# XinShuo-ph/gaussian_splatting_with_eye_tracking

Hardware: AMD Instinct MI355X
Metric: rendered views/sec (fwd+bwd) at 1080p, 1M Gaussians; achieved HBM GB/s % (higher is better)
Workload: dtype fp32; 1 GPU

## Files before the change

gaussian_splatting_with_eye_tracking_amd/csrc/gs_api.cpp:

```cpp
#include <hip/hip_runtime.h>

#include <atomic>
#include <cstdio>
#include <cstdlib>
#include <chrono>
#include <cstring>
#include <functional>
#include <algorithm>
#include <deque>
#include <mutex>
#include <stdexcept>
#include <string>
#include <unordered_set>
#include <utility>
#include <vector>

#include "../../include/gsplat_amd.h"
#include "gs_kernels.h"
#include "gs_layout.h"

using namespace gsamd;

namespace {

// ... 310 lines not shown
    in.store_cov3d = t_store_cov3d != 0;
    in.fwd_zero = t_fwd_zero != 0 && grad;
    in.step0_unfilled = amr && t_amr_step0_unfilled != 0;
    if (amr) t_amr_step0_unfilled = 0;
    return in;
}

PreprocessArgs make_pp(const ForwardIn& in, int tile) {
    PreprocessArgs a;
    a.P = in.P;
    a.D = in.D;
    a.M = in.M;
    a.means3D = in.means3D;
    a.scales = in.scales;
    a.scale_modifier = in.scale_modifier;
    a.rotations = in.rotations;
    a.opacities = in.opacities;
    a.shs = in.shs;
    a.cov3D_precomp = in.cov3D_precomp;
    a.colors_precomp = in.colors_precomp;
    a.viewmatrix = in.viewmatrix;
    a.projmatrix = in.projmatrix;
    a.cam_pos = in.cam_pos;
    a.W = in.width;
    a.H = in.height;
    a.tan_fovx = in.tan_fovx;
    a.tan_fovy = in.tan_fovy;
    a.focal_y = (float)in.height / (2.0f * in.tan_fovy);
    a.focal_x = (float)in.width / (2.0f * in.tan_fovx);
    a.block = tile;
    a.prefiltered = in.prefiltered;
    a.store_cov3d = in.store_cov3d;
    a.store_drgb = in.store_drgb;
    a.zero_words = nullptr;
    a.zero_n = 0;
    a.err_token = 0;
    a.antialiasing = in.antialiasing;
    return a;
}

struct Binned {
    GeomView g;
    ImageView img;
    BinningView b;
    AmrBinningView ab;
    int K;
    int T;
    int* radii;
};

int tile_count(int W, int H, int tile) { return ((W + tile - 1) / tile) * ((H + tile - 1) / tile); }

ImageView image_view(char* image, int W, int H, int tile) {
    ImageView v;
    carve_image(image, (size_t)W * H, tile_count(W, H, tile), &v, tile);
    return v;
}

Binned carve_buffers(char* geom, char* binning, char* image, int P, int K, int W, int H, int tile,
                     bool amr = false) {
    Binned r{};
    r.K = K;
    r.T = tile_count(W, H, tile);
    carve_geom(geom, P, &r.g);
    r.img = image_view(image, W, H, tile);
    carve_binning(binning, K, &r.b, amr ? &r.ab : nullptr);
    r.radii = r.g.radii;
    return r;
}

int rendered_count(int hint, char* geom, int P, const char* binning, hipStream_t s, const char* missing) {
    int K = hint;
    if (K < 0) {
        GeomView g;
        carve_geom(geom, P, &g);
        uint32_t hdr[4];
        read_header(g.hdr, hdr, s);
        K = (int)hdr[kHdrNumRendered];
    }
    if (K > 0 && !binning) throw GsError(missing);
    return K;
}

Binned preprocess_and_bin(const ForwardIn& in, const gs_buffer& geometry, const gs_buffer& binning,
                          const gs_buffer& image, int* radii, int tile, bool debug, hipStream_t s,
                          const std::function<void(Binned&)>& before_k = nullptr, int fused_sort_max = 0) {
    Binned r;
    const int W = in.width, H = in.height;
    const int gx = (W + tile - 1) / tile, gy = (H + tile - 1) / tile;
    r.T = gx * gy;
    const size_t N = (size_t)W * H;
    const bool tail = in.store_cov3d || (in.colors_precomp == nullptr && in.store_drgb);
    char* gbase = call_resize(geometry, carve_geom(nullptr, in.P, nullptr, tail, tile == 32), "geometry");
    carve_geom(gbase, in.P, &r.g);
    set_accum_clean(r.g.grad_accum, false);
    char* ibase = call_resize(image, carve_image(nullptr, N, r.T, nullptr, tile), "image");
    carve_image(ibase, N, r.T, &r.img, tile);
    r.radii = radii ? radii : r.g.radii;
    const bool lds_bin = r.T <= kLdsTiles;
    if (r.T == 0) GS_HIP(hipMemsetAsync(r.g.hdr, 0, kHdrWords * sizeof(uint32_t), s));
    if (r.T > 0 && !lds_bin) GS_HIP(hipMemsetAsync(r.img.tile_count, 0, sizeof(uint32_t) * kBinSlots * r.T, s));
    PreprocessArgs pa = make_pp(in, tile);
    pa.err_token = next_error_token();
    set_drgb_written(r.g.drgb, pa.store_drgb && in.colors_precomp == nullptr);
    if (r.T > 0 && lds_bin) {
        pa.zero_words = r.img.tile_count;
        pa.zero_n = kBinSlots * r.T;
    }
    { StageTimer _t(kPre, s); launch_preprocess(pa, r.g, r.radii, lds_bin ? nullptr : r.img.tile_count, s); }
    stage_check(debug, s, "preprocess");
    if (lds_bin) { StageTimer _t(kCount, s); launch_count_tiles(in.P, r.g, r.radii, W, H, tile, r.img, s); }
    stage_check(debug, s, "count_tiles");
    const std::pair<uint32_t*, uint32_t*> mirror =
        (r.T > 0 && hdr_mirror_on()) ? mirror_words() : std::pair<uint32_t*, uint32_t*>{nullptr, nullptr};
    const bool amr = tile == 32;
    bool dup_done = false;
    const SpecKey skey = spec_key(W, H, in.P);
    const size_t cap = (!amr && !before_k && r.T > 0 && !debug) ? spec_capacity(skey) : 0;
    const uint32_t mtoken = mirror.second ? next_mirror_token() : 0u;
    const bool pub_dup = cap > 0 && mirror.second != nullptr;
    if (r.T > 0) { StageTimer _t(kScan, s); launch_tile_scan(r.T, r.img, r.g.hdr, s, pub_dup ? nullptr : mirror.second, bin_slots_for(in.P, gx, gy, tile), gx, dup_banded(gx, gy, tile), pub_dup ? 0u : mtoken); }
    stage_check(debug, s, "tile_scan");
    uint32_t hdr[4];
    if (before_k) {
        begin_header_read(r.g.hdr, s, mirror.first);
        before_k(r);
        finish_header_read(hdr, mirror.first, s, r.g.hdr);
    } else if (cap > 0) {
        begin_header_read(r.g.hdr, s, mirror.first);
        char* sbase = call_resize(binning, carve_binning(nullptr, cap, nullptr), "binning");
        carve_binning(sbase, cap, &r.b);
        { StageTimer _t(kDup, s); launch_duplicate(in.P, r.g, r.radii, W, H, tile, r.img, r.b, s, (uint32_t)cap, r.g.hdr, (uint32_t)cap, pub_dup ? mirror.second : nullptr, pub_dup ? mtoken : 0u); }
        finish_header_read(hdr, mirror.first, s, r.g.hdr);
        dup_done = hdr[kHdrNumRendered] <= cap;
    } else if (mirror.first) {
        begin_header_read(r.g.hdr, s, mirror.first);
        finish_header_read(hdr, mirror.first, s, r.g.hdr);
    } else {
        read_header(r.g.hdr, hdr, s);
    }
    if (in.prefiltered && hdr[kHdrError] == pa.err_token)
        throw GsError("Point is filtered although prefiltered is set. This shouldn't happen!");
    r.K = (int)hdr[kHdrNumRendered];
    if (!amr) note_k(skey, r.K);
    if (!dup_done) {
        char* bbase = call_resize(binning, carve_binning(nullptr, r.K, nullptr, nullptr, amr), "binning");
        carve_binning(bbase, r.K, &r.b, amr ? &r.ab : nullptr);
    }
    if (r.K > 0) {
        if (!dup_done) { StageTimer _t(kDup, s); launch_duplicate(in.P, r.g, r.radii, W, H, tile, r.img, r.b, s, (uint32_t)r.K); }
        stage_check(debug, s, "duplicate");
        { StageTimer _t(kSort, s); launch_sort_tiles(r.T, r.img, r.b, (int)hdr[kHdrMaxTileCount], (int)hdr[kHdrNumLargeTiles], s, fused_sort_max); }
        stage_check(debug, s, "sort_tiles");
    }
    return r;
}

}

DispatchEvents gsamd::take_dispatch_events() {
    const DispatchEvents e = t_dispatch;
    t_dispatch = DispatchEvents{};
    return e;
}

extern "C" {

int gs_abi_version(void) { return GSPLAT_AMD_ABI_VERSION; }

#ifndef GSAMD_DIGEST
#define GSAMD_DIGEST "unstamped"
#endif
const char* gs_build_digest(void) { return GSAMD_DIGEST; }

const char* gs_last_error(void) { return g_err.c_str(); }

namespace {
int base_forward_impl(const ForwardIn& in, const gs_buffer& geometry, const gs_buffer& binning,
                      const gs_buffer& image, float* out_color, int* radii, bool aux, float* out_depth,
                      float* out_alpha, int debug, void* stream, const char* who) {
    const int P = in.P, width = in.width, height = in.height;
    if (aux && (!out_depth || !out_alpha)) throw GsError(std::string(who) + ": out_depth / out_alpha is NULL");
    hipStream_t s = static_cast<hipStream_t>(stream);
    if (P <= 0) {
        if (aux) {
            const size_t N = (width > 0 && height > 0) ? (size_t)width * (size_t)height : 0;
            if (N) {
                GS_HIP(hipMemsetAsync(out_depth, 0, sizeof(float) * N, s));
                GS_HIP(hipMemsetAsync(out_alpha, 0, sizeof(float) * N, s));
            }
        }
        return 0;
    }
    Binned r = preprocess_and_bin(in, geometry, binning, image, radii, 16, debug != 0, s);
    const float* feats = in.colors_precomp ? in.colors_precomp : r.g.rgb;
    bool zeroed;
    {
        StageTimer _t(kRender, s, true);
        const bool zero = in.fwd_zero;
        zeroed = launch_render_forward(width, height, r.img, r.b, r.g, feats, in.background, out_color, s,
                                       zero ? r.g.grad_accum : nullptr, zero ? (size_t)kGradRow * (size_t)P : 0,
                                       reinterpret_cast<uint8_t*>(r.b.scratch));
    }
    if (zeroed) set_accum_clean(r.g.grad_accum, true);
    stage_check(debug != 0, s, "render");
    if (aux) {
        launch_render_forward_aux(width, height, r.img, r.b, r.g, out_depth, out_alpha, s);
        stage_check(debug != 0, s, "render_aux");
    }
    return r.K;
}
}

int gs_rasterizer_forward(gs_buffer geometry, gs_buffer binning, gs_buffer image, int P, int D, int M,
                          const float* background, int width, int height, const float* means3D, const float* shs,
                          const float* colors_precomp, const float* opacities, const float* scales,
                          float scale_modifier, const float* rotations, const float* cov3D_precomp,
                          const float* viewmatrix, const float* projmatrix, const float* cam_pos, float tan_fovx,
                          float tan_fovy, int prefiltered, float* out_color, int* radii, int debug, void* stream) {
    const ForwardIn in = forward_in(false, P, D, M, background, width, height, means3D, shs, colors_precomp, opacities,
                                    scales, scale_modifier, rotations, cov3D_precomp, viewmatrix, projmatrix, cam_pos,
                                    tan_fovx, tan_fovy, prefiltered);
    return guarded([&]() -> int {
        return base_forward_impl(in, geometry, binning, image, out_color, radii, false, nullptr, nullptr, debug,
                                 stream, "gs_rasterizer_forward");
    });
}

int gs_rasterizer_forward_aux(gs_buffer geometry, gs_buffer binning, gs_buffer image, int P, int D, int M,
                              const float* background, int width, int height, const float* means3D, const float* shs,
                              const float* colors_precomp, const float* opacities, const float* scales,
                              float scale_modifier, const float* rotations, const float* cov3D_precomp,
                              const float* viewmatrix, const float* projmatrix, const float* cam_pos, float tan_fovx,
                              float tan_fovy, int prefiltered, float* out_color, int* radii, float* out_depth,
                              float* out_alpha, int debug, void* stream) {
    const ForwardIn in = forward_in(false, P, D, M, background, width, height, means3D, shs, colors_precomp, opacities,
                                    scales, scale_modifier, rotations, cov3D_precomp, viewmatrix, projmatrix, cam_pos,
// ... 773 lines not shown
    });
}

int gs_l1_ssim_loss(const float* image, const float* gt, int C, int H, int W, float lambda_dssim, float* grad,
                    float* out3, gs_buffer workspace, void* stream) {
    return guarded([&]() -> int {
        if (C <= 0 || H <= 0 || W <= 0) return 0;
        hipStream_t s = static_cast<hipStream_t>(stream);
        char* ws = call_resize(workspace, l1_ssim_workspace_bytes(C, H, W), "loss workspace");
        launch_l1_ssim(image, gt, C, H, W, lambda_dssim, grad, out3, reinterpret_cast<float*>(ws), s);
        stage_check(false, s, "l1_ssim");
        return 0;
    });
}

int gs_adam_step(float* params, const float* grads, float* exp_avg, float* exp_avg_sq, long long n, int nseg,
                 const long long* seg_end, const double* lr, const long long* step, double beta1, double beta2, double eps,
                 void* stream) {
    return guarded([&]() -> int {
        if (nseg < 1 || nseg > 8) throw GsError("gs_adam_step: 1..8 segments");
        for (int i = 0; i < nseg; i++)
            if (step[i] < 0 || (i > 0 && seg_end[i] < seg_end[i - 1])) throw GsError("gs_adam_step: bad segments");
        hipStream_t s = static_cast<hipStream_t>(stream);
        launch_adam(params, grads, exp_avg, exp_avg_sq, n, nseg, seg_end, lr, step, beta1, beta2, eps, s);
        stage_check(false, s, "adam");
        return 0;
    });
}

int gs_densify_stats(int P, const int* radii, const float* grad_means2D, int grad_stride, float* xyz_gradient_accum,
                     float* denom, float* max_radii2D, void* stream) {
    return guarded([&]() -> int {
        if (P < 0 || grad_stride < 2) throw GsError("gs_densify_stats: bad sizes");
        hipStream_t s = static_cast<hipStream_t>(stream);
        launch_densify_stats(P, radii, grad_means2D, grad_stride, xyz_gradient_accum, denom, max_radii2D, s);
        stage_check(false, s, "densify_stats");
        return 0;
    });
}

int gs_activate_gaussians(int P, int M, const float* features_dc, const float* features_rest, const float* opacity_raw,
                          const float* scaling_raw, const float* rotation_raw, float* shs, float* opacities,
                          float* scales, float* rotations, void* stream) {
    return guarded([&]() -> int {
        if (P < 0 || M < 1 || M > 16) throw GsError("gs_activate_gaussians: bad sizes");
        hipStream_t s = static_cast<hipStream_t>(stream);
        launch_activate(P, M, features_dc, features_rest, opacity_raw, scaling_raw, rotation_raw, shs, opacities,
                        scales, rotations, s);
        stage_check(false, s, "activate");
        return 0;
    });
}

int gs_activation_backward(int P, int M, int accumulate, const float* dL_dshs, const float* dL_dopacities,
                           const float* dL_dscales, const float* dL_drotations, const float* dL_dmeans3D,
                           const float* opacity_raw, const float* scaling_raw, const float* rotation_raw,
                           float* grad_xyz, float* grad_features_dc, float* grad_features_rest, float* grad_opacity,
                           float* grad_scaling, float* grad_rotation, void* stream) {
    return guarded([&]() -> int {
        if (P < 0 || M < 1 || M > 16) throw GsError("gs_activation_backward: bad sizes");
        hipStream_t s = static_cast<hipStream_t>(stream);
        launch_activation_backward(P, M, accumulate, dL_dshs, dL_dopacities, dL_dscales, dL_drotations, dL_dmeans3D,
                                   opacity_raw, scaling_raw, rotation_raw, grad_xyz, grad_features_dc,
                                   grad_features_rest, grad_opacity, grad_scaling, grad_rotation, s);
        stage_check(false, s, "activation_backward");
        return 0;
    });
}

namespace {
struct TuningKey {
    const char* key;
    const int* value;
    void (*set)(int);
};
const TuningKey kTuning[] = {
    {"fwd_variant", &g_fwd_variant, set_forward_variant},
    {"bwd_variant", &g_bwd_variant, set_backward_variant},
    {"amr_variant", &g_amr_variant, set_amr_variant},
    {"sort_algo", &g_sort_algo, set_sort_algo},
    {"cull", &g_cull, set_cull},
    {"hdr_mirror", &g_hdr_mirror, [](int v) { g_hdr_mirror = v == 0 ? 0 : 2; }},
    {"spec_dup", &g_spec_dup, [](int v) { g_spec_dup = v; }},
    {"ritnet_mfma", &g_ritnet_mfma, set_ritnet_mfma},
};

const TuningKey* tuning_key(const char* key) {
    for (const TuningKey& e : kTuning)
        if (key && std::strcmp(key, e.key) == 0) return &e;
    if (key) g_err = std::string("unknown tuning key ") + key;
    return nullptr;
}
}

int gs_set_tuning(const char* key, int value) {
    const TuningKey* e = tuning_key(key);
    if (e) e->set(value);
    return e ? 0 : -1;
}

int gs_get_tuning(const char* key, int* value) {
    if (!key || !value) return -1;
    hdr_mirror_on();
    const TuningKey* e = tuning_key(key);
    if (!e) return -1;
    *value = *e->value;
    return 0;
}

int gs_set_thread_option(const char* key, int value) {
    if (!key) return -1;
    const struct { const char* key; int* value; } table[] = {{"fwd_no_grad", &t_fwd_no_grad},
                                                             {"sh_drgb", &t_sh_drgb},
                                                             {"store_cov3d", &t_store_cov3d},
                                                             {"fwd_zero", &t_fwd_zero},
                                                             {"amr_step0_unfilled", &t_amr_step0_unfilled}};
    for (const auto& e : table)
        if (std::strcmp(key, e.key) == 0) {
            *e.value = value;
            return 0;
        }
    g_err = std::string("unknown thread option ") + key;
    return -1;
}

void gs_profile_enable(int on) {
    std::lock_guard<std::mutex> l(g_prof_mu);
    g_prof.on = on != 0;
}

void gs_profile_set_mask(unsigned mask) {
    std::lock_guard<std::mutex> l(g_prof_mu);
    g_prof.mask = mask;
}

int gs_profile_stage_count(void) { return kStages; }

const char* gs_profile_stage_name(int i) { return (i >= 0 && i < kStages) ? kStageNames[i] : ""; }

void gs_profile_read(double* total_ms, long* counts, int reset) {
    std::lock_guard<std::mutex> l(g_prof_mu);
    g_prof.harvest();
    for (int i = 0; i < kStages; i++) {
        if (total_ms) total_ms[i] = g_prof.total_ms[i];
        if (counts) counts[i] = g_prof.count[i];
        if (reset) {
            g_prof.total_ms[i] = 0;
            g_prof.count[i] = 0;
        }
    }
}

size_t gs_geom_bytes(int P) { return carve_geom(nullptr, (size_t)P, nullptr); }

size_t gs_amr_geom_bytes(int P) { return carve_geom(nullptr, (size_t)P, nullptr, true, true); }

size_t gs_image_bytes(int width, int height, int tile) {
    return carve_image(nullptr, (size_t)width * height, tile_count(width, height, tile), nullptr, tile);
}

size_t gs_binning_bytes(int K) { return carve_binning(nullptr, (size_t)K, nullptr); }

namespace {
int binning_count_of_bytes(size_t nbytes, bool amr) {
    long lo = 0, hi = (long)std::min<size_t>(nbytes / 8 + 1, (size_t)INT32_MAX);
    while (lo < hi) {
// ... 51 lines not shown
```

gaussian_splatting_with_eye_tracking_amd/csrc/gs_kernels.h:

```cpp
#pragma once

#include <hip/hip_runtime.h>
#include <stdint.h>

#include "gs_layout.h"

namespace gsamd {

struct DispatchEvents {
    hipEvent_t start = nullptr, stop = nullptr;
};
DispatchEvents take_dispatch_events();

struct PreprocessArgs {
    int P, D, M;
    const float* means3D;
    const float* scales;
    float scale_modifier;
    const float* rotations;
    const float* opacities;
    const float* shs;
    const float* cov3D_precomp;
    const float* colors_precomp;
    const float* viewmatrix;
    const float* projmatrix;
    const float* cam_pos;
    int W, H;
    float tan_fovx, tan_fovy, focal_x, focal_y;
    int block;
    int prefiltered;
    int store_cov3d;
    int store_drgb;
    uint32_t* zero_words;
    int zero_n;
    uint32_t err_token;
    int antialiasing = 0;
};

void launch_preprocess(const PreprocessArgs& a, const GeomView& g, int* radii, uint32_t* tile_count,
                       hipStream_t s);
void launch_mark_visible(int P, const float* means3D, const float* viewmatrix, const float* projmatrix,
                         bool* present, hipStream_t s);

void launch_tile_scan(int T, const ImageView& img, uint32_t* hdr, hipStream_t s, uint32_t* hdr_mirror, int nslots,
                      int gx, bool banded, uint32_t mirror_token = 0);
void launch_duplicate(int P, const GeomView& g, const int* radii, int W, int H, int block, const ImageView& img,
                      const BinningView& b, hipStream_t s, uint32_t n_keys, const uint32_t* spec_hdr = nullptr,
                      uint32_t spec_cap = 0, uint32_t* mirror = nullptr, uint32_t mirror_token = 0);
constexpr int kLdsTiles = 16384;
void launch_count_tiles(int P, const GeomView& g, const int* radii, int W, int H, int block, const ImageView& img,
                        hipStream_t s);
void set_sort_algo(int v);
int bin_slots_for(int P, int gx, int gy, int block);
bool dup_banded(int gx, int gy, int block);
void launch_order_tiles(int T, const ImageView& img, bool use_max_contrib, hipStream_t s);
void launch_sort_tiles(int T, const ImageView& img, const BinningView& b, int max_count_host, int num_large_host,
                       hipStream_t s, int fused_max = 0);
constexpr int kAmrFusedSortMax = 2048;
constexpr int kAmrStepsAll = GSPLAT_AMD_AMR_STEPS_1_TO_4;
constexpr int kAmrStepsAllFill = GSPLAT_AMD_AMR_STEPS_1_TO_4_FILL;
constexpr int kAmrStepsAllSplit = GSPLAT_AMD_AMR_STEPS_1_TO_4_SPLIT;
constexpr int kAmrStateAfter = 100;
bool fused_sort_on();
void launch_reconstruct_keys(int T, const ImageView& img, const BinningView& b, const GeomView& g, uint64_t* keys,
                             hipStream_t s);

bool launch_render_forward(int W, int H, const ImageView& img, const BinningView& b, const GeomView& g,
                           const float* features, const float* bg, float* out_color, hipStream_t s,
                           float* zero_rows = nullptr, size_t zero_floats = 0, uint8_t* hit_codes = nullptr);
void launch_render_forward_aux(int W, int H, const ImageView& img, const BinningView& b, const GeomView& g,
                               float* out_depth, float* out_alpha, hipStream_t s);
void launch_render_backward_aux(int W, int H, const ImageView& img, const BinningView& b, const GeomView& g,
                                const float* colors, const float* bg, const float* dL_dpix, const float* dL_ddepth,
                                const float* dL_dalpha, hipStream_t s);
void launch_aux_depth_to_means(int P, const GeomView& g, const int* radii, const float* viewmatrix,
                               float* dL_dmean3D, hipStream_t s);
void set_forward_variant(int v);
void set_backward_variant(int v);
void set_amr_variant(int v);
void set_cull(int v);
void set_ritnet_mfma(int v);
void launch_render_backward(int W, int H, const ImageView& img, const BinningView& b, const GeomView& g,
                            const float* colors, const float* bg, const float* dL_dpix, hipStream_t s, int K);
constexpr int kDetRow = 9;
void launch_render_backward_deterministic(int W, int H, int P, int R, const ImageView& img, const BinningView& b,
                                          const GeomView& g, const int* radii, const float* colors, const float* bg,
                                          const float* dL_dpix, float* partials, uint32_t err_token, hipStream_t s);

struct BackwardGaussArgs {
    int P, D, M;
    const float* means3D;
    const int* radii;
    const float* shs;
    const float* scales;
    const float* rotations;
    float scale_modifier;
    const float* cov3D;
    const float* viewmatrix;
    const float* projmatrix;
    const float* campos;
    float focal_x, focal_y, tan_fovx, tan_fovy;
    int has_cov_precomp;
    const float* drgb;
    const uint32_t* hdr;
    int drgb_known;
    int nt_out = 0;
    const float* opacities = nullptr;
    int antialiasing = 0;
    uint32_t* err_word = nullptr;
    uint32_t err_token = 0;
    float* dL_dmean2D;
    float* dL_dconic;
    float* dL_dopacity;
    float* dL_dcolor;
    float* dL_dmean3D;
    float* dL_dcov3D;
    float* dL_dsh;
    float* dL_dscale;
    float* dL_drot;
};
void launch_backward_gaussians(const BackwardGaussArgs& a, const GeomView& g, hipStream_t s);

constexpr int kViewRow = 10;
// ... 82 lines not shown
```

gaussian_splatting_with_eye_tracking_amd/csrc/preprocess.hip:

```cpp
#include <algorithm>

#include "gs_blend.cuh"
#include "gs_device.cuh"
#include "gs_kernels.h"

namespace gsamd {

template <bool kSH16>
__device__ __forceinline__ void load_sh(int deg, int M, const float* __restrict__ sh, float (&c)[16][3]) {
    const int ncoef = min((deg + 1) * (deg + 1), M);
    if (kSH16) {
        const float4* s4 = reinterpret_cast<const float4*>(sh);
        float buf[48];
#pragma unroll
        for (int i = 0; i < 12; i++) {
            const float4 v = (i * 4 < ncoef * 3) ? s4[i] : make_float4(0.f, 0.f, 0.f, 0.f);
            buf[4 * i + 0] = v.x; buf[4 * i + 1] = v.y; buf[4 * i + 2] = v.z; buf[4 * i + 3] = v.w;
        }
#pragma unroll
        for (int k = 0; k < 16; k++)
#pragma unroll
            for (int ch = 0; ch < 3; ch++) c[k][ch] = buf[3 * k + ch];
    } else {
#pragma unroll
        for (int k = 0; k < 16; k++)
#pragma unroll
            for (int ch = 0; ch < 3; ch++) c[k][ch] = (k < ncoef) ? sh[3 * k + ch] : 0.f;
    }
}

__device__ __forceinline__ float3 eval_sh_color(int deg, const float (&c)[16][3], float x, float y, float z,
                                                uint8_t& clamped_bits) {
    float res[3];
#pragma unroll
    for (int ch = 0; ch < 3; ch++) res[ch] = SH_C0 * c[0][ch];
    if (deg > 0) {
        const float k1 = SH_C1 * y, k2 = SH_C1 * z, k3 = SH_C1 * x;
#pragma unroll
        for (int ch = 0; ch < 3; ch++) res[ch] = res[ch] - k1 * c[1][ch] + k2 * c[2][ch] - k3 * c[3][ch];
        if (deg > 1) {
            const float xx = x * x, yy = y * y, zz = z * z;
            const float xy = x * y, yz = y * z, xz = x * z;
            const float k4 = SH_C2_0 * xy;
            const float k5 = SH_C2_1 * yz;
            const float k6 = SH_C2_2 * (2.0f * zz - xx - yy);
            const float k7 = SH_C2_3 * xz;
            const float k8 = SH_C2_4 * (xx - yy);
#pragma unroll
            for (int ch = 0; ch < 3; ch++)
                res[ch] = res[ch] + k4 * c[4][ch] + k5 * c[5][ch] + k6 * c[6][ch] + k7 * c[7][ch] + k8 * c[8][ch];
            if (deg > 2) {
                const float k9 = SH_C3_0 * y * (3.0f * xx - yy);
                const float k10 = SH_C3_1 * xy * z;
                const float k11 = SH_C3_2 * y * (4.0f * zz - xx - yy);
                const float k12 = SH_C3_3 * z * (2.0f * zz - 3.0f * xx - 3.0f * yy);
                const float k13 = SH_C3_4 * x * (4.0f * zz - xx - yy);
                const float k14 = SH_C3_5 * z * (xx - yy);
                const float k15 = SH_C3_6 * x * (xx - 3.0f * yy);
#pragma unroll
                for (int ch = 0; ch < 3; ch++)
                    res[ch] = res[ch] + k9 * c[9][ch] + k10 * c[10][ch] + k11 * c[11][ch] + k12 * c[12][ch] +
                              k13 * c[13][ch] + k14 * c[14][ch] + k15 * c[15][ch];
            }
        }
    }
    clamped_bits = 0;
#pragma unroll
    for (int ch = 0; ch < 3; ch++) {
        res[ch] += 0.5f;
        if (res[ch] < 0) clamped_bits |= (uint8_t)(1u << ch);
        res[ch] = fmaxf(res[ch], 0.0f);
    }
    return make_float3(res[0], res[1], res[2]);
}

constexpr int kPpThreads = 256;
constexpr int kShStride = 52;

template <bool kHasSH, bool kCovPrecomp, bool kAA, typename ShFn>
__device__ __forceinline__ void pp_gaussian(const PreprocessArgs& a, const GeomView& g, int* __restrict__ radii,
                                            uint32_t* __restrict__ tile_count, int idx, bool radii_copy, float mx,
                                            float my, float mz, const float (&sc)[3], float4 q, float (&cov3D)[6],
                                            float opacity, const Mat4& V, const Mat4& Pm, ShFn&& load_shc,
                                            float* stage) {
    const float3 p_view = transform_point_4x3(mx, my, mz, V);
    if (p_view.z <= 0.2f) {
        if (a.prefiltered) g.hdr[kHdrError] = a.err_token;
        return;
    }
    const float4 p_hom = transform_point_4x4(mx, my, mz, Pm);
    const float p_w = 1.0f / (p_hom.w + 0.0000001f);
    const float p_proj_x = p_hom.x * p_w;
    const float p_proj_y = p_hom.y * p_w;

    if (!kCovPrecomp) {
        compute_cov3d(sc, q, a.scale_modifier, cov3D);
        if (a.store_cov3d) {
#pragma unroll
            for (int i = 0; i < 6; i++) g.cov3D[6 * idx + i] = cov3D[i];
        }
    }

    float3 t = transform_point_4x3(mx, my, mz, V);
    const float limx = 1.3f * a.tan_fovx;
    const float limy = 1.3f * a.tan_fovy;
    const float txtz = t.x / t.z;
    const float tytz = t.y / t.z;
    t.x = fminf(limx, fmaxf(-limx, txtz)) * t.z;
    t.y = fminf(limy, fmaxf(-limy, tytz)) * t.z;
    const Mat3 J = mat3_cols(a.focal_x / t.z, 0.0f, -(a.focal_x * t.x) / (t.z * t.z), 0.0f, a.focal_y / t.z,
                             -(a.focal_y * t.y) / (t.z * t.z), 0, 0, 0);
    const float* v = V.m;
    const Mat3 Wm = mat3_cols(v[0], v[4], v[8], v[1], v[5], v[9], v[2], v[6], v[10]);
    const Mat3 T = mat3_mul(Wm, J);
    const Mat3 Vrk = mat3_cols(cov3D[0], cov3D[1], cov3D[2], cov3D[1], cov3D[3], cov3D[4], cov3D[2], cov3D[4],
                               cov3D[5]);
    Mat3 cov = mat3_mul(mat3_mul(mat3_transpose(T), mat3_transpose(Vrk)), T);
    float det0 = 0.f;
    if constexpr (kAA) det0 = cov.m[0][0] * cov.m[1][1] - cov.m[0][1] * cov.m[0][1];
    cov.m[0][0] += 0.3f;
    cov.m[1][1] += 0.3f;
    const float cx = cov.m[0][0], cy = cov.m[0][1], cz = cov.m[1][1];

    const float det = (cx * cz - cy * cy);
    if (det == 0.0f) return;
    if constexpr (kAA) opacity = opacity * sqrtf(fmaxf(0.000025f, det0 / det));
    const float det_inv = 1.f / det;
    const float conic_x = cz * det_inv, conic_y = -cy * det_inv, conic_z = cx * det_inv;
    const float mid = 0.5f * (cx + cz);
    const float lambda1 = mid + sqrtf(fmaxf(0.1f, mid * mid - det));
    const float lambda2 = mid - sqrtf(fmaxf(0.1f, mid * mid - det));
    const float my_radius = ceilf(3.f * sqrtf(fmaxf(lambda1, lambda2)));
    const float pix_x = ndc2pix(p_proj_x, a.W);
    const float pix_y = ndc2pix(p_proj_y, a.H);
    const uint32_t gx = (uint32_t)((a.W + a.block - 1) / a.block);
    const uint32_t gy = (uint32_t)((a.H + a.block - 1) / a.block);
    const int iradius = (int)my_radius;
    const Rect r = get_rect(pix_x, pix_y, iradius, a.block, a.block, gx, gy);
    const uint32_t area = (r.x1 - r.x0) * (r.y1 - r.y0);
    if (area == 0) return;

    float3 rgbv = make_float3(0.f, 0.f, 0.f);
    if (kHasSH) {
        float shc[16][3];
        load_shc(shc);
        float dx = mx - a.cam_pos[0], dy = my - a.cam_pos[1], dz = mz - a.cam_pos[2];
        const float len = sqrtf(dot3(dx, dy, dz, dx, dy, dz));
        dx = dx / len; dy = dy / len; dz = dz / len;
        uint8_t cbits;
        const float3 rgb = eval_sh_color(a.D, shc, dx, dy, dz, cbits);
        if (a.store_drgb) {
            float dx3[3], dy3[3], dz3[3];
            sh_ddir(a.D, shc, dx, dy, dz, dx3, dy3, dz3);
            float4* row = stage ? reinterpret_cast<float4*>(stage)
                                : reinterpret_cast<float4*>(g.drgb) + 3 * (size_t)idx;
            row[0] = make_float4(dx3[0], dx3[1], dx3[2], dy3[0]);
            row[1] = make_float4(dy3[1], dy3[2], dz3[0], dz3[1]);
            row[2] = make_float4(dz3[2], 0.f, 0.f, 0.f);
        }
        if (stage) {
            *reinterpret_cast<float4*>(stage + 12) = make_float4(rgb.x, rgb.y, rgb.z, 0.f);
        } else {
            g.rgb[3 * idx + 0] = rgb.x;
            g.rgb[3 * idx + 1] = rgb.y;
            g.rgb[3 * idx + 2] = rgb.z;
        }
        rgbv = rgb;
        g.clamped[idx] = cbits;
    }
    g.depths[idx] = p_view.z;
    radii[idx] = iradius;
    if (radii_copy) g.radii[idx] = iradius;
    reinterpret_cast<float2*>(g.means2D)[idx] = make_float2(pix_x, pix_y);
    reinterpret_cast<float4*>(g.conic_opacity)[idx] = make_float4(conic_x, conic_y, conic_z, opacity);
    g.tiles_touched[idx] = area;
    if (a.block == 32) {
        float r_, g_, b_;
        if (kHasSH) {
            r_ = rgbv.x; g_ = rgbv.y; b_ = rgbv.z;
        } else {
            r_ = a.colors_precomp[3 * idx]; g_ = a.colors_precomp[3 * idx + 1]; b_ = a.colors_precomp[3 * idx + 2];
        }
        float4* row = stage ? reinterpret_cast<float4*>(stage + 16)
                            : reinterpret_cast<float4*>(g.amr_rows + (size_t)16 * idx);
        const float4 co = make_float4(conic_x, conic_y, conic_z, opacity);
        row[0] = make_float4(pix_x, pix_y, r_, g_);
        row[1] = splat_coef(co);
        row[2] = make_float4(b_, conic_x, conic_y, conic_z);
        if (!stage) row[3] = make_float4(0.f, 0.f, 0.f, 0.f);
    }

    if (tile_count)
        for (uint32_t y = r.y0; y < r.y1; y++)
            for (uint32_t x = r.x0; x < r.x1; x++) atomicAdd(&tile_count[y * gx + x], 1u);
}

template <bool kHasSH, bool kSH16, bool kCovPrecomp, bool kDma, bool kNtIn = false, bool kAA = false>
__device__ __forceinline__ void pp_thread(const PreprocessArgs& a, const GeomView& g, int* __restrict__ radii,
                                          uint32_t* __restrict__ tile_count, int idx, const float* sh_row,
                                          float* stage) {
    const bool radii_copy = a.block == 32 && radii != g.radii;
    radii[idx] = 0;
    if (radii_copy) g.radii[idx] = 0;
    g.tiles_touched[idx] = 0;

    const float mx = ldg1<kNtIn>(a.means3D + 3 * idx + 0);
    const float my = ldg1<kNtIn>(a.means3D + 3 * idx + 1);
    const float mz = ldg1<kNtIn>(a.means3D + 3 * idx + 2);
    float sc[3] = {0.f, 0.f, 0.f};
    float4 q = make_float4(0.f, 0.f, 0.f, 0.f);
    float cov3D[6];
    if (kCovPrecomp) {
#pragma unroll
        for (int i = 0; i < 6; i++) cov3D[i] = a.cov3D_precomp[6 * idx + i];
    } else {
        sc[0] = ldg1<kNtIn>(a.scales + 3 * idx + 0);
        sc[1] = ldg1<kNtIn>(a.scales + 3 * idx + 1);
        sc[2] = ldg1<kNtIn>(a.scales + 3 * idx + 2);
        q = ldg4<kNtIn>(reinterpret_cast<const float4*>(a.rotations) + idx);
    }
    const float opacity = ldg1<kNtIn>(a.opacities + idx);
    const Mat4 V = load_mat4(a.viewmatrix);
    const Mat4 Pm = load_mat4(a.projmatrix);
    pp_gaussian<kHasSH, kCovPrecomp, kAA>(a, g, radii, tile_count, idx, radii_copy, mx, my, mz, sc, q, cov3D, opacity,
                                     V, Pm, [&](float (&shc)[16][3]) {
        if constexpr (kDma) {
            asm volatile("s_waitcnt vmcnt(0)" ::: "memory");
            const int ncoef = min((a.D + 1) * (a.D + 1), a.M);
            typedef float f4v __attribute__((ext_vector_type(4)));
            float v[48];
#pragma unroll
            for (int i = 0; i < 12; i++) {
                f4v t = reinterpret_cast<const f4v*>(sh_row)[i];
                asm volatile("" : "+v"(t));
                v[4 * i] = t.x; v[4 * i + 1] = t.y; v[4 * i + 2] = t.z; v[4 * i + 3] = t.w;
            }
#pragma unroll
            for (int k = 0; k < 16; k++)
#pragma unroll
                for (int ch = 0; ch < 3; ch++) shc[k][ch] = k < ncoef ? v[3 * k + ch] : 0.f;
        } else {
            load_sh<kSH16>(a.D, a.M, a.shs + (size_t)idx * a.M * 3, shc);
        }
    }, stage);
}

template <bool kHasSH, bool kSH16, bool kCovPrecomp, bool kDma = false, bool kAA = false>
__global__ void __launch_bounds__(kPpThreads) preprocess_kernel(PreprocessArgs a, GeomView g, int* __restrict__ radii,
                                                                uint32_t* __restrict__ tile_count) {
    static_assert(!kDma || (kHasSH && kSH16), "LDS-DMA stages 16-coefficient SH rows");
    constexpr bool kStageOut = kDma, kNtIn = kDma;
    const int idx = blockIdx.x * blockDim.x + threadIdx.x;
    __shared__ __attribute__((aligned(16))) float s_sh[kDma ? kPpThreads * kShStride : 1];
    if constexpr (kDma) {
        const int w = threadIdx.x >> 6, lane = threadIdx.x & 63;
        const size_t row0 = (size_t)blockIdx.x * kPpThreads + 64 * w;
        const float* src = a.shs + row0 * 48;
        float* dst = s_sh + 64 * kShStride * w;
        constexpr int kPieces = kShStride / 4;
#pragma unroll
        for (int i = 0; i < kPieces; i++) {
            const int p = 64 * i + lane, r = p / kPieces, j = p - kPieces * r;
            if (j < 12 && row0 + (size_t)r < (size_t)a.P)
                __builtin_amdgcn_global_load_lds(src + 48 * r + 4 * j, dst + 256 * i, 16, 0, 2);
        }
    }
    for (int i = idx; i < a.zero_n; i += (int)(gridDim.x * blockDim.x)) a.zero_words[i] = 0u;
    if (idx == 0) g.hdr[kHdrDrgb] = (kHasSH && a.store_drgb) ? 1u : 0u;
    if (idx == 0) g.hdr[kHdrAntialias] = kAA ? 1u : 0u;
    float* row = s_sh + (kDma ? kShStride * threadIdx.x : 0);
    if constexpr (kStageOut) {
        const int wrow0 = (int)(blockIdx.x * kPpThreads) + (int)(threadIdx.x & ~63u);
        if (wrow0 >= a.P) return;
        if (idx < a.P) pp_thread<kHasSH, kSH16, kCovPrecomp, kDma, kNtIn, kAA>(a, g, radii, tile_count, idx, row, row);
        __builtin_amdgcn_fence(__ATOMIC_RELEASE, "wavefront");
        __builtin_amdgcn_wave_barrier();
        __builtin_amdgcn_fence(__ATOMIC_ACQUIRE, "wavefront");
        const int lane = threadIdx.x & 63;
        const float* wl = s_sh + kShStride * (threadIdx.x & ~63u);
        const int nrow = min(64, a.P - wrow0);
        if (a.store_drgb) {
            float4* out = reinterpret_cast<float4*>(g.drgb) + 3 * (size_t)wrow0;
#pragma unroll
            for (int i = 0; i < 3; i++) {
                const int c = lane + 64 * i;
                if (c < 3 * nrow) {
                    const float4 v = *reinterpret_cast<const float4*>(wl + kShStride * (c / 3) + 4 * (c % 3));
                    typedef float f4v __attribute__((ext_vector_type(4)));
                    __builtin_nontemporal_store(f4v{v.x, v.y, v.z, v.w}, reinterpret_cast<f4v*>(out + c));
                }
            }
        }
        if (a.block == 32) {
            float4* out = reinterpret_cast<float4*>(g.amr_rows + (size_t)16 * wrow0);
#pragma unroll
            for (int i = 0; i < 4; i++) {
                const int c = lane + 64 * i;
                if (c < 4 * nrow)
                    out[c] = (c & 3) == 3 ? make_float4(0.f, 0.f, 0.f, 0.f)
                                          : *reinterpret_cast<const float4*>(wl + kShStride * (c >> 2) + 16 + 4 * (c & 3));
            }
        }
        const int nf = 3 * nrow;
        if (4 * lane < nf) {
            float v4[4];
#pragma unroll
            for (int e = 0; e < 4; e++) {
                const int f = min(4 * lane + e, nf - 1);
                v4[e] = wl[kShStride * (f / 3) + 12 + f % 3];
            }
            float* out = g.rgb + 3 * (size_t)wrow0 + 4 * lane;
            if (4 * lane + 4 <= nf) {
                *reinterpret_cast<float4*>(out) = make_float4(v4[0], v4[1], v4[2], v4[3]);
            } else {
#pragma unroll
                for (int e = 0; e < 3; e++)
                    if (4 * lane + e < nf) out[e] = v4[e];
            }
        }
        return;
    }
    if (idx >= a.P) return;
    pp_thread<kHasSH, kSH16, kCovPrecomp, kDma, false, kAA>(a, g, radii, tile_count, idx, row, nullptr);
}

template <bool A, bool B, bool C>
static void launch_pp(const PreprocessArgs& a, const GeomView& g, int* radii, uint32_t* tile_count, hipStream_t s) {
    const int blocks = (a.P + kPpThreads - 1) / kPpThreads;
    if (a.antialiasing && a.block == 16)
        hipLaunchKernelGGL((preprocess_kernel<A, B, C, A && B, true>), dim3(blocks), dim3(kPpThreads), 0, s, a, g,
                           radii, tile_count);
    else
        hipLaunchKernelGGL((preprocess_kernel<A, B, C, A && B>), dim3(blocks), dim3(kPpThreads), 0, s, a, g, radii,
                           tile_count);
}

void launch_preprocess(const PreprocessArgs& a, const GeomView& g, int* radii, uint32_t* tile_count,
                       hipStream_t s) {
    if (a.P == 0) return;
    const bool has_sh = a.colors_precomp == nullptr;
    const bool sh16 = has_sh && a.M == 16;
    const bool covp = a.cov3D_precomp != nullptr;
    if (has_sh) {
        if (sh16) {
            if (covp) launch_pp<true, true, true>(a, g, radii, tile_count, s);
            else launch_pp<true, true, false>(a, g, radii, tile_count, s);
        } else {
            if (covp) launch_pp<true, false, true>(a, g, radii, tile_count, s);
            else launch_pp<true, false, false>(a, g, radii, tile_count, s);
        }
    } else {
        if (covp) launch_pp<false, false, true>(a, g, radii, tile_count, s);
        else launch_pp<false, false, false>(a, g, radii, tile_count, s);
    }
}

__global__ void __launch_bounds__(256) mark_visible_kernel(int P, const float* __restrict__ means3D,
                                                           const float* __restrict__ viewmatrix,
                                                           bool* __restrict__ present) {
    const int idx = blockIdx.x * blockDim.x + threadIdx.x;
    if (idx >= P) return;
    const Mat4 V = load_mat4(viewmatrix);
    const float3 pv = transform_point_4x3(means3D[3 * idx], means3D[3 * idx + 1], means3D[3 * idx + 2], V);
    present[idx] = !(pv.z <= 0.2f);
}

void launch_mark_visible(int P, const float* means3D, const float* viewmatrix, const float* projmatrix,
                         bool* present, hipStream_t s) {
    (void)projmatrix;
    if (P == 0) return;
    hipLaunchKernelGGL(mark_visible_kernel, dim3((P + 255) / 256), dim3(256), 0, s, P, means3D, viewmatrix,
                       present);
}

}
```

Measured before the change: 1275 views/s.

## Split preprocess into geometry and SH-color kernels, overlap color on side stream

Preprocess is split into a geometry kernel (projection, conic, radii, tile footprint) and a persistent SH color kernel. By default the color kernel runs on a side stream and overlaps with tile counting, scan, duplicate and sort, joining before the function returns. The color kernel only loads SH rows for visible Gaussians via an LDS DMA ballot, which skips SH reads for culled points. In exchange it adds stream and event management, a second pass over means3D and radii, and possible contention with the binning kernels.

```diff
diff --git a/gaussian_splatting_with_eye_tracking_amd/csrc/gs_api.cpp b/gaussian_splatting_with_eye_tracking_amd/csrc/gs_api.cpp
--- a/gaussian_splatting_with_eye_tracking_amd/csrc/gs_api.cpp
+++ b/gaussian_splatting_with_eye_tracking_amd/csrc/gs_api.cpp
@@ -416,6 +416,71 @@
     return K;
 }
 
+constexpr int kPpOverlapDefault = 2;
+int g_pp_overlap = kPpOverlapDefault;
+
+struct SideStream {
+    int dev = -1;
+    hipStream_t launch = nullptr, side = nullptr;
+    hipEvent_t fork = nullptr, join = nullptr;
+    uint64_t used = 0;
+};
+constexpr int kSideEntries = 16;
+thread_local SideStream t_side[kSideEntries];
+thread_local uint64_t t_side_clock = 0;
+
+SideStream& side_stream_for(hipStream_t launch) {
+    int dev = 0;
+    GS_HIP(hipGetDevice(&dev));
+    SideStream* lru = &t_side[0];
+    for (SideStream& e : t_side) {
+        if (e.side && e.dev == dev && e.launch == launch) {
+            e.used = ++t_side_clock;
+            return e;
+        }
+        if (e.used < lru->used) lru = &e;
+    }
+    SideStream& e = *lru;
+    if (e.side) {
+        int cur = dev;
+        if (e.dev != dev) GS_HIP_NOTHROW(hipSetDevice(e.dev));
+        GS_HIP_NOTHROW(hipStreamSynchronize(e.side));
+        GS_HIP_NOTHROW(hipStreamDestroy(e.side));
+        GS_HIP_NOTHROW(hipEventDestroy(e.fork));
+        GS_HIP_NOTHROW(hipEventDestroy(e.join));
+        if (e.dev != dev) GS_HIP_NOTHROW(hipSetDevice(cur));
+        e = SideStream{};
+    }
+    SideStream n;
+    GS_HIP(hipStreamCreateWithFlags(&n.side, hipStreamNonBlocking));
+    if (hipEventCreateWithFlags(&n.fork, hipEventDisableTiming) != hipSuccess ||
+        hipEventCreateWithFlags(&n.join, hipEventDisableTiming) != hipSuccess) {
+        if (n.fork) GS_HIP_NOTHROW(hipEventDestroy(n.fork));
+        GS_HIP_NOTHROW(hipStreamDestroy(n.side));
+        throw GsError("pp_overlap: could not create the side stream's events");
+    }
+    n.dev = dev;
+    n.launch = launch;
+    n.used = ++t_side_clock;
+    e = n;
+    return e;
+}
+
+struct ColorJoin {
+    hipStream_t s = nullptr;
+    hipEvent_t ev = nullptr;
+    void arm(hipStream_t launch, hipEvent_t join) { s = launch; ev = join; }
+    void wait() {
+        if (!ev) return;
+        hipEvent_t e = ev;
+        ev = nullptr;
+        GS_HIP(hipStreamWaitEvent(s, e, 0));
+    }
+    ~ColorJoin() {
+        if (ev) GS_HIP_NOTHROW(hipStreamWaitEvent(s, ev, 0));
+    }
+};
+
 Binned preprocess_and_bin(const ForwardIn& in, const gs_buffer& geometry, const gs_buffer& binning,
                           const gs_buffer& image, int* radii, int tile, bool debug, hipStream_t s,
                           const std::function<void(Binned&)>& before_k = nullptr, int fused_sort_max = 0) {
@@ -441,7 +506,28 @@
         pa.zero_words = r.img.tile_count;
         pa.zero_n = kBinSlots * r.T;
     }
-    { StageTimer _t(kPre, s); launch_preprocess(pa, r.g, r.radii, lds_bin ? nullptr : r.img.tile_count, s); }
+    const int pp_mode = (lds_bin && r.T > 0 && preprocess_splits(pa)) ? g_pp_overlap : 0;
+    const bool pp_timed = g_prof.on && ((g_prof.mask >> kPre) & 1u);
+    const bool pp_side = pp_mode == 2 && !debug && !pp_timed;
+    ColorJoin join;
+    if (pp_mode == 0) {
+        StageTimer _t(kPre, s);
+        launch_preprocess(pa, r.g, r.radii, lds_bin ? nullptr : r.img.tile_count, s);
+    } else {
+        {
+            StageTimer _t(kPre, s);
+            launch_preprocess_geom(pa, r.g, r.radii, s);
+            if (!pp_side) launch_preprocess_color(pa, r.g, r.radii, s, false);
+        }
+        if (pp_side) {
+            SideStream& ss = side_stream_for(s);
+            GS_HIP(hipEventRecord(ss.fork, s));
+            GS_HIP(hipStreamWaitEvent(ss.side, ss.fork, 0));
+            launch_preprocess_color(pa, r.g, r.radii, ss.side, true);
+            GS_HIP(hipEventRecord(ss.join, ss.side));
+            join.arm(s, ss.join);
+        }
+    }
     stage_check(debug, s, "preprocess");
     if (lds_bin) { StageTimer _t(kCount, s); launch_count_tiles(in.P, r.g, r.radii, W, H, tile, r.img, s); }
     stage_check(debug, s, "count_tiles");
@@ -487,6 +573,7 @@
         { StageTimer _t(kSort, s); launch_sort_tiles(r.T, r.img, r.b, (int)hdr[kHdrMaxTileCount], (int)hdr[kHdrNumLargeTiles], s, fused_sort_max); }
         stage_check(debug, s, "sort_tiles");
     }
+    join.wait();
     return r;
 }
 
@@ -1426,6 +1513,7 @@
     {"cull", &g_cull, set_cull},
     {"hdr_mirror", &g_hdr_mirror, [](int v) { g_hdr_mirror = v == 0 ? 0 : 2; }},
     {"spec_dup", &g_spec_dup, [](int v) { g_spec_dup = v; }},
+    {"pp_overlap", &g_pp_overlap, [](int v) { g_pp_overlap = (v < 0 || v > 2) ? kPpOverlapDefault : v; }},
     {"ritnet_mfma", &g_ritnet_mfma, set_ritnet_mfma},
 };
 
diff --git a/gaussian_splatting_with_eye_tracking_amd/csrc/gs_kernels.h b/gaussian_splatting_with_eye_tracking_amd/csrc/gs_kernels.h
--- a/gaussian_splatting_with_eye_tracking_amd/csrc/gs_kernels.h
+++ b/gaussian_splatting_with_eye_tracking_amd/csrc/gs_kernels.h
@@ -39,6 +39,10 @@
 
 void launch_preprocess(const PreprocessArgs& a, const GeomView& g, int* radii, uint32_t* tile_count,
                        hipStream_t s);
+bool preprocess_splits(const PreprocessArgs& a);
+void launch_preprocess_geom(const PreprocessArgs& a, const GeomView& g, int* radii, hipStream_t s);
+void launch_preprocess_color(const PreprocessArgs& a, const GeomView& g, const int* radii, hipStream_t s,
+                             bool beside);
 void launch_mark_visible(int P, const float* means3D, const float* viewmatrix, const float* projmatrix,
                          bool* present, hipStream_t s);
 
diff --git a/gaussian_splatting_with_eye_tracking_amd/csrc/preprocess.hip b/gaussian_splatting_with_eye_tracking_amd/csrc/preprocess.hip
--- a/gaussian_splatting_with_eye_tracking_amd/csrc/preprocess.hip
+++ b/gaussian_splatting_with_eye_tracking_amd/csrc/preprocess.hip
@@ -1,4 +1,5 @@
 #include <algorithm>
+#include <atomic>
 
 #include "gs_blend.cuh"
 #include "gs_device.cuh"
@@ -77,16 +78,21 @@
 constexpr int kPpThreads = 256;
 constexpr int kShStride = 52;
 
-template <bool kHasSH, bool kCovPrecomp, bool kAA, typename ShFn>
-__device__ __forceinline__ void pp_gaussian(const PreprocessArgs& a, const GeomView& g, int* __restrict__ radii,
-                                            uint32_t* __restrict__ tile_count, int idx, bool radii_copy, float mx,
-                                            float my, float mz, const float (&sc)[3], float4 q, float (&cov3D)[6],
-                                            float opacity, const Mat4& V, const Mat4& Pm, ShFn&& load_shc,
-                                            float* stage) {
+struct PpGeom {
+    float depth, pix_x, pix_y, conic_x, conic_y, conic_z, opacity;
+    int iradius;
+    Rect r;
+    uint32_t area, gx;
+};
+
+template <bool kCovPrecomp, bool kAA>
+__device__ __forceinline__ bool pp_geometry(const PreprocessArgs& a, const GeomView& g, int idx, float mx, float my,
+                                            float mz, const float (&sc)[3], float4 q, float (&cov3D)[6],
+                                            float opacity, const Mat4& V, const Mat4& Pm, PpGeom& o) {
     const float3 p_view = transform_point_4x3(mx, my, mz, V);
     if (p_view.z <= 0.2f) {
         if (a.prefiltered) g.hdr[kHdrError] = a.err_token;
-        return;
+        return false;
     }
     const float4 p_hom = transform_point_4x4(mx, my, mz, Pm);
     const float p_w = 1.0f / (p_hom.w + 0.0000001f);
@@ -123,57 +129,80 @@
     const float cx = cov.m[0][0], cy = cov.m[0][1], cz = cov.m[1][1];
 
     const float det = (cx * cz - cy * cy);
-    if (det == 0.0f) return;
+    if (det == 0.0f) return false;
     if constexpr (kAA) opacity = opacity * sqrtf(fmaxf(0.000025f, det0 / det));
     const float det_inv = 1.f / det;
-    const float conic_x = cz * det_inv, conic_y = -cy * det_inv, conic_z = cx * det_inv;
+    o.conic_x = cz * det_inv; o.conic_y = -cy * det_inv; o.conic_z = cx * det_inv;
     const float mid = 0.5f * (cx + cz);
     const float lambda1 = mid + sqrtf(fmaxf(0.1f, mid * mid - det));
     const float lambda2 = mid - sqrtf(fmaxf(0.1f, mid * mid - det));
     const float my_radius = ceilf(3.f * sqrtf(fmaxf(lambda1, lambda2)));
-    const float pix_x = ndc2pix(p_proj_x, a.W);
-    const float pix_y = ndc2pix(p_proj_y, a.H);
-    const uint32_t gx = (uint32_t)((a.W + a.block - 1) / a.block);
+    o.pix_x = ndc2pix(p_proj_x, a.W);
+    o.pix_y = ndc2pix(p_proj_y, a.H);
+    o.gx = (uint32_t)((a.W + a.block - 1) / a.block);
     const uint32_t gy = (uint32_t)((a.H + a.block - 1) / a.block);
-    const int iradius = (int)my_radius;
-    const Rect r = get_rect(pix_x, pix_y, iradius, a.block, a.block, gx, gy);
-    const uint32_t area = (r.x1 - r.x0) * (r.y1 - r.y0);
-    if (area == 0) return;
-
+    o.iradius = (int)my_radius;
+    o.r = get_rect(o.pix_x, o.pix_y, o.iradius, a.block, a.block, o.gx, gy);
+    o.area = (o.r.x1 - o.r.x0) * (o.r.y1 - o.r.y0);
+    if (o.area == 0) return false;
+    o.depth = p_view.z;
+    o.opacity = opacity;
+    return true;
+}
+
+__device__ __forceinline__ void pp_geom_store(const GeomView& g, int* __restrict__ radii, int idx, bool radii_copy,
+                                              const PpGeom& o) {
+    g.depths[idx] = o.depth;
+    radii[idx] = o.iradius;
+    if (radii_copy) g.radii[idx] = o.iradius;
+    reinterpret_cast<float2*>(g.means2D)[idx] = make_float2(o.pix_x, o.pix_y);
+    reinterpret_cast<float4*>(g.conic_opacity)[idx] = make_float4(o.conic_x, o.conic_y, o.conic_z, o.opacity);
+    g.tiles_touched[idx] = o.area;
+}
+
+template <typename ShFn>
+__device__ __forceinline__ float3 pp_color(const PreprocessArgs& a, const GeomView& g, int idx, float mx, float my,
+                                           float mz, ShFn&& load_shc, float* stage) {
+    float shc[16][3];
+    load_shc(shc);
+    float dx = mx - a.cam_pos[0], dy = my - a.cam_pos[1], dz = mz - a.cam_pos[2];
+    const float len = sqrtf(dot3(dx, dy, dz, dx, dy, dz));
+    dx = dx / len; dy = dy / len; dz = dz / len;
+    uint8_t cbits;
+    const float3 rgb = eval_sh_color(a.D, shc, dx, dy, dz, cbits);
+    if (a.store_drgb) {
+        float dx3[3], dy3[3], dz3[3];
+        sh_ddir(a.D, shc, dx, dy, dz, dx3, dy3, dz3);
+        float4* row = stage ? reinterpret_cast<float4*>(stage)
+                            : reinterpret_cast<float4*>(g.drgb) + 3 * (size_t)idx;
+        row[0] = make_float4(dx3[0], dx3[1], dx3[2], dy3[0]);
+        row[1] = make_float4(dy3[1], dy3[2], dz3[0], dz3[1]);
+        row[2] = make_float4(dz3[2], 0.f, 0.f, 0.f);
+    }
+    if (stage) {
+        *reinterpret_cast<float4*>(stage + 12) = make_float4(rgb.x, rgb.y, rgb.z, 0.f);
+    } else {
+        g.rgb[3 * idx + 0] = rgb.x;
+        g.rgb[3 * idx + 1] = rgb.y;
+        g.rgb[3 * idx + 2] = rgb.z;
+    }
+    g.clamped[idx] = cbits;
+    return rgb;
+}
+
+template <bool kHasSH, bool kCovPrecomp, bool kAA, typename ShFn>
+__device__ __forceinline__ void pp_gaussian(const PreprocessArgs& a, const GeomView& g, int* __restrict__ radii,
+                                            uint32_t* __restrict__ tile_count, int idx, bool radii_copy, float mx,
+                                            float my, float mz, const float (&sc)[3], float4 q, float (&cov3D)[6],
+                                            float opacity, const Mat4& V, const Mat4& Pm, ShFn&& load_shc,
+                                            float* stage) {
+    PpGeom o;
+    if (!pp_geometry<kCovPrecomp, kAA>(a, g, idx, mx, my, mz, sc, q, cov3D, opacity, V, Pm, o)) return;
     float3 rgbv = make_float3(0.f, 0.f, 0.f);
-    if (kHasSH) {
-        float shc[16][3];
-        load_shc(shc);
-        float dx = mx - a.cam_pos[0], dy = my - a.cam_pos[1], dz = mz - a.cam_pos[2];
-        const float len = sqrtf(dot3(dx, dy, dz, dx, dy, dz));
-        dx = dx / len; dy = dy / len; dz = dz / len;
-        uint8_t cbits;
-        const float3 rgb = eval_sh_color(a.D, shc, dx, dy, dz, cbits);
-        if (a.store_drgb) {
-            float dx3[3], dy3[3], dz3[3];
-            sh_ddir(a.D, shc, dx, dy, dz, dx3, dy3, dz3);
-            float4* row = stage ? reinterpret_cast<float4*>(stage)
-                                : reinterpret_cast<float4*>(g.drgb) + 3 * (size_t)idx;
-            row[0] = make_float4(dx3[0], dx3[1], dx3[2], dy3[0]);
-            row[1] = make_float4(dy3[1], dy3[2], dz3[0], dz3[1]);
-            row[2] = make_float4(dz3[2], 0.f, 0.f, 0.f);
-        }
-        if (stage) {
-            *reinterpret_cast<float4*>(stage + 12) = make_float4(rgb.x, rgb.y, rgb.z, 0.f);
-        } else {
-            g.rgb[3 * idx + 0] = rgb.x;
-            g.rgb[3 * idx + 1] = rgb.y;
-            g.rgb[3 * idx + 2] = rgb.z;
-        }
-        rgbv = rgb;
-        g.clamped[idx] = cbits;
-    }
-    g.depths[idx] = p_view.z;
-    radii[idx] = iradius;
-    if (radii_copy) g.radii[idx] = iradius;
-    reinterpret_cast<float2*>(g.means2D)[idx] = make_float2(pix_x, pix_y);
-    reinterpret_cast<float4*>(g.conic_opacity)[idx] = make_float4(conic_x, conic_y, conic_z, opacity);
-    g.tiles_touched[idx] = area;
+    if (kHasSH) rgbv = pp_color(a, g, idx, mx, my, mz, load_shc, stage);
+    pp_geom_store(g, radii, idx, radii_copy, o);
+    const float pix_x = o.pix_x, pix_y = o.pix_y, conic_x = o.conic_x, conic_y = o.conic_y, conic_z = o.conic_z;
+    const float opacity_rec = o.opacity;
     if (a.block == 32) {
         float r_, g_, b_;
         if (kHasSH) {
@@ -183,7 +212,7 @@
         }
         float4* row = stage ? reinterpret_cast<float4*>(stage + 16)
                             : reinterpret_cast<float4*>(g.amr_rows + (size_t)16 * idx);
-        const float4 co = make_float4(conic_x, conic_y, conic_z, opacity);
+        const float4 co = make_float4(conic_x, conic_y, conic_z, opacity_rec);
         row[0] = make_float4(pix_x, pix_y, r_, g_);
         row[1] = splat_coef(co);
         row[2] = make_float4(b_, conic_x, conic_y, conic_z);
@@ -191,8 +220,8 @@
     }
 
     if (tile_count)
-        for (uint32_t y = r.y0; y < r.y1; y++)
-            for (uint32_t x = r.x0; x < r.x1; x++) atomicAdd(&tile_count[y * gx + x], 1u);
+        for (uint32_t y = o.r.y0; y < o.r.y1; y++)
+            for (uint32_t x = o.r.x0; x < o.r.x1; x++) atomicAdd(&tile_count[y * o.gx + x], 1u);
 }
 
 template <bool kHasSH, bool kSH16, bool kCovPrecomp, bool kDma, bool kNtIn = false, bool kAA = false>
@@ -243,6 +272,52 @@
             load_sh<kSH16>(a.D, a.M, a.shs + (size_t)idx * a.M * 3, shc);
         }
     }, stage);
+}
+
+__device__ __forceinline__ void pp_store_wave_records(const PreprocessArgs& a, const GeomView& g, const float* s_sh,
+                                                      int wrow0) {
+    const int lane = threadIdx.x & 63;
+    const float* wl = s_sh + kShStride * (threadIdx.x & ~63u);
+    const int nrow = min(64, a.P - wrow0);
+    if (a.store_drgb) {
+        float4* out = reinterpret_cast<float4*>(g.drgb) + 3 * (size_t)wrow0;
+#pragma unroll
+        for (int i = 0; i < 3; i++) {
+            const int c = lane + 64 * i;
+            if (c < 3 * nrow) {
+                const float4 v = *reinterpret_cast<const float4*>(wl + kShStride * (c / 3) + 4 * (c % 3));
+                typedef float f4v __attribute__((ext_vector_type(4)));
+                __builtin_nontemporal_store(f4v{v.x, v.y, v.z, v.w}, reinterpret_cast<f4v*>(out + c));
+            }
+        }
+    }
+    if (a.block == 32) {
+        float4* out = reinterpret_cast<float4*>(g.amr_rows + (size_t)16 * wrow0);
+#pragma unroll
+        for (int i = 0; i < 4; i++) {
+            const int c = lane + 64 * i;
+            if (c < 4 * nrow)
+                out[c] = (c & 3) == 3 ? make_float4(0.f, 0.f, 0.f, 0.f)
+                                      : *reinterpret_cast<const float4*>(wl + kShStride * (c >> 2) + 16 + 4 * (c & 3));
+        }
+    }
+    const int nf = 3 * nrow;
+    if (4 * lane < nf) {
+        float v4[4];
+#pragma unroll
+        for (int e = 0; e < 4; e++) {
+            const int f = min(4 * lane + e, nf - 1);
+            v4[e] = wl[kShStride * (f / 3) + 12 + f % 3];
+        }
+        float* out = g.rgb + 3 * (size_t)wrow0 + 4 * lane;
+        if (4 * lane + 4 <= nf) {
+            *reinterpret_cast<float4*>(out) = make_float4(v4[0], v4[1], v4[2], v4[3]);
+        } else {
+#pragma unroll
+            for (int e = 0; e < 3; e++)
+                if (4 * lane + e < nf) out[e] = v4[e];
+        }
+    }
 }
 
 template <bool kHasSH, bool kSH16, bool kCovPrecomp, bool kDma = false, bool kAA = false>
@@ -276,52 +351,128 @@
         __builtin_amdgcn_fence(__ATOMIC_RELEASE, "wavefront");
         __builtin_amdgcn_wave_barrier();
         __builtin_amdgcn_fence(__ATOMIC_ACQUIRE, "wavefront");
-        const int lane = threadIdx.x & 63;
-        const float* wl = s_sh + kShStride * (threadIdx.x & ~63u);
-        const int nrow = min(64, a.P - wrow0);
-        if (a.store_drgb) {
-            float4* out = reinterpret_cast<float4*>(g.drgb) + 3 * (size_t)wrow0;
-#pragma unroll
-            for (int i = 0; i < 3; i++) {
-                const int c = lane + 64 * i;
-                if (c < 3 * nrow) {
-                    const float4 v = *reinterpret_cast<const float4*>(wl + kShStride * (c / 3) + 4 * (c % 3));
-                    typedef float f4v __attribute__((ext_vector_type(4)));
-                    __builtin_nontemporal_store(f4v{v.x, v.y, v.z, v.w}, reinterpret_cast<f4v*>(out + c));
-                }
-            }
-        }
-        if (a.block == 32) {
-            float4* out = reinterpret_cast<float4*>(g.amr_rows + (size_t)16 * wrow0);
-#pragma unroll
-            for (int i = 0; i < 4; i++) {
-                const int c = lane + 64 * i;
-                if (c < 4 * nrow)
-                    out[c] = (c & 3) == 3 ? make_float4(0.f, 0.f, 0.f, 0.f)
-                                          : *reinterpret_cast<const float4*>(wl + kShStride * (c >> 2) + 16 + 4 * (c & 3));
-            }
-        }
-        const int nf = 3 * nrow;
-        if (4 * lane < nf) {
-            float v4[4];
-#pragma unroll
-            for (int e = 0; e < 4; e++) {
-                const int f = min(4 * lane + e, nf - 1);
-                v4[e] = wl[kShStride * (f / 3) + 12 + f % 3];
-            }
-            float* out = g.rgb + 3 * (size_t)wrow0 + 4 * lane;
-            if (4 * lane + 4 <= nf) {
-                *reinterpret_cast<float4*>(out) = make_float4(v4[0], v4[1], v4[2], v4[3]);
-            } else {
-#pragma unroll
-                for (int e = 0; e < 3; e++)
-                    if (4 * lane + e < nf) out[e] = v4[e];
-            }
-        }
+        pp_store_wave_records(a, g, s_sh, wrow0);
         return;
     }
     if (idx >= a.P) return;
     pp_thread<kHasSH, kSH16, kCovPrecomp, kDma, false, kAA>(a, g, radii, tile_count, idx, row, nullptr);
+}
+
+template <bool kAA>
+__global__ void __launch_bounds__(kPpThreads) preprocess_geom_kernel(PreprocessArgs a, GeomView g,
+                                                                     int* __restrict__ radii) {
+    const int idx = blockIdx.x * blockDim.x + threadIdx.x;
+    for (int i = idx; i < a.zero_n; i += (int)(gridDim.x * blockDim.x)) a.zero_words[i] = 0u;
+    if (idx == 0) g.hdr[kHdrDrgb] = a.store_drgb ? 1u : 0u;
+    if (idx == 0) g.hdr[kHdrAntialias] = kAA ? 1u : 0u;
+    if (idx >= a.P) return;
+    radii[idx] = 0;
+    g.tiles_touched[idx] = 0;
+    const float mx = ldg1<true>(a.means3D + 3 * idx + 0);
+    const float my = ldg1<true>(a.means3D + 3 * idx + 1);
+    const float mz = ldg1<true>(a.means3D + 3 * idx + 2);
+    float sc[3];
+    sc[0] = ldg1<true>(a.scales + 3 * idx + 0);
+    sc[1] = ldg1<true>(a.scales + 3 * idx + 1);
+    sc[2] = ldg1<true>(a.scales + 3 * idx + 2);
+    const float4 q = ldg4<true>(reinterpret_cast<const float4*>(a.rotations) + idx);
+    const float opacity = ldg1<true>(a.opacities + idx);
+    const Mat4 V = load_mat4(a.viewmatrix);
+    const Mat4 Pm = load_mat4(a.projmatrix);
+    float cov3D[6];
+    PpGeom o;
+    if (pp_geometry<false, kAA>(a, g, idx, mx, my, mz, sc, q, cov3D, opacity, V, Pm, o))
+        pp_geom_store(g, radii, idx, false, o);
+}
+
+constexpr int kColorThreads = 64;
+__global__ void __launch_bounds__(kColorThreads)
+preprocess_color_kernel(PreprocessArgs a, GeomView g, const int* __restrict__ radii) {
+    __shared__ __attribute__((aligned(16))) float s_sh[kColorThreads * kShStride];
+    const int lane = threadIdx.x;
+    const int nchunk = (a.P + 63) / 64;
+    float* row = s_sh + kShStride * lane;
+    int c = (int)blockIdx.x;
+    if (c >= nchunk) return;
+    int rad = (64 * c + lane < a.P) ? radii[64 * c + lane] : 0;
+    for (; c < nchunk; c += (int)gridDim.x) {
+        const int wrow0 = 64 * c, idx = wrow0 + lane;
+        const bool vis = rad > 0;
+        const unsigned long long live = __ballot(vis);
+        const int cn = c + (int)gridDim.x;
+        if (cn < nchunk) rad = (64 * cn + lane < a.P) ? radii[64 * cn + lane] : 0;
+        if (live == 0ull) continue;
+        {
+            const float* src = a.shs + (size_t)wrow0 * 48;
+            constexpr int kPieces = kShStride / 4;
+#pragma unroll
+            for (int i = 0; i < kPieces; i++) {
+                const int p = 64 * i + lane, r = p / kPieces, j = p - kPieces * r;
+                if (j < 12 && ((live >> r) & 1ull))
+                    __builtin_amdgcn_global_load_lds(src + 48 * r + 4 * j, s_sh + 256 * i, 16, 0, 2);
+            }
+        }
+        if (vis) {
+            const float mx = a.means3D[3 * idx + 0];
+            const float my = a.means3D[3 * idx + 1];
+            const float mz = a.means3D[3 * idx + 2];
+            pp_color(a, g, idx, mx, my, mz, [&](float (&shc)[16][3]) {
+                asm volatile("s_waitcnt vmcnt(0)" ::: "memory");
+                const int ncoef = min((a.D + 1) * (a.D + 1), a.M);
+                typedef float f4v __attribute__((ext_vector_type(4)));
+                float v[48];
+#pragma unroll
+                for (int i = 0; i < 12; i++) {
+                    f4v t = reinterpret_cast<const f4v*>(row)[i];
+                    asm volatile("" : "+v"(t));
+                    v[4 * i] = t.x; v[4 * i + 1] = t.y; v[4 * i + 2] = t.z; v[4 * i + 3] = t.w;
+                }
+#pragma unroll
+                for (int k = 0; k < 16; k++)
+#pragma unroll
+                    for (int ch = 0; ch < 3; ch++) shc[k][ch] = k < ncoef ? v[3 * k + ch] : 0.f;
+            }, row);
+        }
+        __builtin_amdgcn_fence(__ATOMIC_RELEASE, "wavefront");
+        __builtin_amdgcn_wave_barrier();
+        __builtin_amdgcn_fence(__ATOMIC_ACQUIRE, "wavefront");
+        pp_store_wave_records(a, g, s_sh, wrow0);
+        asm volatile("s_waitcnt lgkmcnt(0)" ::: "memory");
+        __builtin_amdgcn_wave_barrier();
+    }
+}
+
+bool preprocess_splits(const PreprocessArgs& a) {
+    return a.P > 0 && a.colors_precomp == nullptr && a.M == 16 && a.cov3D_precomp == nullptr && a.block == 16;
+}
+
+void launch_preprocess_geom(const PreprocessArgs& a, const GeomView& g, int* radii, hipStream_t s) {
+    const int blocks = (a.P + kPpThreads - 1) / kPpThreads;
+    if (a.antialiasing)
+        hipLaunchKernelGGL(preprocess_geom_kernel<true>, dim3(blocks), dim3(kPpThreads), 0, s, a, g, radii);
+    else
+        hipLaunchKernelGGL(preprocess_geom_kernel<false>, dim3(blocks), dim3(kPpThreads), 0, s, a, g, radii);
+}
+
+static int device_cus() {
+    constexpr int kMaxDev = 64;
+    static std::atomic<int> cus[kMaxDev];
+    int dev = 0;
+    if (hipGetDevice(&dev) != hipSuccess || dev < 0 || dev >= kMaxDev) return 256;
+    int v = cus[dev].load(std::memory_order_relaxed);
+    if (v == 0) {
+        if (hipDeviceGetAttribute(&v, hipDeviceAttributeMultiprocessorCount, dev) != hipSuccess || v <= 0) v = 256;
+        cus[dev].store(v, std::memory_order_relaxed);
+    }
+    return v;
+}
+
+constexpr int kColorWavesBeside = 4, kColorWavesAlone = 8;
+void launch_preprocess_color(const PreprocessArgs& a, const GeomView& g, const int* radii, hipStream_t s,
+                             bool beside) {
+    const int nchunk = (a.P + 63) / 64;
+    const int blocks = std::min(nchunk, device_cus() * (beside ? kColorWavesBeside : kColorWavesAlone));
+    hipLaunchKernelGGL(preprocess_color_kernel, dim3(blocks), dim3(kColorThreads), 0, s, a, g, radii);
 }
 
 template <bool A, bool B, bool C>
```

Measured after the change: 1287 views/s, median of 6. No clear change (+1.0%).
